# computablee/heterogeneous-spmv

Hardware: AMD Instinct MI355X
Metric: SpMV GFLOP/s and achieved HBM GB/s (fp64) per matrix, 1/2/4/8 MI355X (higher is better)
Workload: dtype f64

## Files before the change

heterogeneous-spmv_amd/csrc/hspmv_options.cpp:

```cpp
#include <string.h>

#include <algorithm>
#include <atomic>
#include <cmath>
#include <cstddef>
#include <cstdlib>
#include <thread>
#include <vector>

#include "hspmv_runtime.h"

namespace hspmv {

int tuning_from_options(const hspmv_options *o, Tuning *t) {
  *t = Tuning();
  if (!o) return HSPMV_OK;
  if (o->struct_size < offsetof(hspmv_options, csr3_plan))
    return set_error(HSPMV_E_INVALID, "hspmv_options.struct_size %u too small", o->struct_size);
  hspmv_options v;
  memset(&v, 0, sizeof(v));
  memcpy(&v, o, std::min<size_t>(o->struct_size, sizeof(v)));
  if (v.csr3_plan < 0 || v.csr3_plan > HSPMV_CSR3_PLAN_SSR)
    return set_error(HSPMV_E_INVALID, "csr3_plan %d unknown", v.csr3_plan);
  if ((v.csort_parts && v.csort_parts != 1 && v.csort_parts != 2 && v.csort_parts != 4) ||
      (v.csort_chunk_u && v.csort_chunk_u != 4 && v.csort_chunk_u != 8 && v.csort_chunk_u != 16) ||
      (v.stream_waves && v.stream_waves != 1 && v.stream_waves != 2 && v.stream_waves != 4) ||
      v.task_nnz < 0 || v.x_dict_cap < 0 || v.placement_trials < 0 || v.placement_trials > 8)
    return set_error(HSPMV_E_INVALID, "hspmv_options: value out of range");
  if (v.deterministic < 0 || v.deterministic > HSPMV_DETERMINISTIC_SERIAL)
    return set_error(HSPMV_E_INVALID, "deterministic %d unknown", v.deterministic);
  if ((v.deterministic == HSPMV_DETERMINISTIC_ORDERED || v.deterministic == HSPMV_DETERMINISTIC_SERIAL) &&
      v.csort > 0)
    return set_error(HSPMV_E_INVALID, "the column-sorted kernel (csort = 1) does not sum in omp_spmv's "
                                      "order (deterministic = 2 runs it with reproducible fixed-point sums)");
  t->csr3_plan = v.csr3_plan;
  t->task_nnz = v.task_nnz;
  t->x_windows = v.x_windows < 0 ? -1 : 0;
  t->x_dict = v.x_dict < 0 ? -1 : (v.x_dict > 0 ? 1 : 0);
  t->x_dict_cap = v.x_dict_cap;
  t->x_slabs = v.x_slabs < 0 ? -1 : v.x_slabs;
  t->col16_group = v.col16_group < 0 ? -1 : (v.col16_group > 0 ? 1 : 0);
  t->csort = v.csort < 0 ? -1 : (v.csort > 0 ? 1 : 0);
  t->csort_parts = v.csort_parts;
  t->csort_u = v.csort_chunk_u;
  t->stream_waves = v.stream_waves;
  t->deterministic = v.deterministic;
  t->placement_trials = v.placement_trials;
  t->row_slices = v.row_slices < 0 ? -1 : (v.row_slices > 0 ? 1 : 0);
  return HSPMV_OK;
}

#ifdef HSPMV_ENV_KNOBS
void tuning_from_env(Tuning *t) {
  auto geti = [](const char *k, int *v) {
    if (const char *e = getenv(k)) *v = atoi(e);
  };
  if (const char *e = getenv("HSPMV_CSR3_PLAN"))
    t->csr3_plan = !strcmp(e, "ssr") ? HSPMV_CSR3_PLAN_SSR
                   : !strcmp(e, "packed") ? HSPMV_CSR3_PLAN_PACKED : HSPMV_CSR3_PLAN_ALIGNED;
  if (const char *e = getenv("HSPMV_TASK_FILL"))
    if (atoi(e) == 0) t->csr3_plan = HSPMV_CSR3_PLAN_PACKED;
  geti("HSPMV_TASK_NNZ", &t->task_nnz);
  if (const char *e = getenv("HSPMV_XWIN")) t->x_windows = atoi(e) == 0 ? -1 : 0;
  if (const char *e = getenv("HSPMV_XDICT")) t->x_dict = atoi(e) == 0 ? -1 : 1;
  geti("HSPMV_XDICT_CAP", &t->x_dict_cap);
  if (const char *e = getenv("HSPMV_XSLABS")) t->x_slabs = atoi(e) == 0 ? -1 : atoi(e);
  if (const char *e = getenv("HSPMV_XSLAB_BYTES")) t->xslab_bytes = atof(e);
  if (const char *e = getenv("HSPMV_COL16G")) t->col16_group = atoi(e) == 0 ? -1 : 1;
  if (const char *e = getenv("HSPMV_CSORT")) t->csort = atoi(e) == 0 ? -1 : 1;
  geti("HSPMV_CSORT_H", &t->csort_parts);
  geti("HSPMV_CSORT_U", &t->csort_u);
// ... 3 lines not shown
  geti("HSPMV_CSORT_SLOT32", &t->csort_slot32);
  geti("HSPMV_CSORT_WIDE", &t->csort_wide);
  geti("HSPMV_CSORT_LDS", &t->csort_lds_cap);
  geti("HSPMV_CSORT_SEG", &t->csort_seg);
  geti("HSPMV_CSORT_SEG_EXTRA", &t->csort_seg_extra);
  geti("HSPMV_CSORT_TRACE", &t->csort_trace);
  geti("HSPMV_CSORT_LONG", &t->csort_long);
  geti("HSPMV_CSORT_BALANCE", &t->csort_balance);
  geti("HSPMV_CSORT_FIN_ROWS", &t->csort_fin_rows);
  geti("HSPMV_CSORT_DYN", &t->csort_dyn);
  if (const char *e = getenv("HSPMV_CSORT_SWEEP")) t->csort_sweep_w = atof(e);
  if (const char *e = getenv("HSPMV_CSORT_SLACK")) t->csort_slack = atof(e);
  geti("HSPMV_CSORT_PART32", &t->csort_part32);
  geti("HSPMV_DETERMINISTIC", &t->deterministic);
  geti("HSPMV_SERIAL_MAX", &t->serial_max);
  geti("HSPMV_LDS_PAD", &t->lds_pad);
  geti("HSPMV_STREAM_W", &t->stream_waves);
  geti("HSPMV_PLACEMENT", &t->placement_trials);
  geti("HSPMV_SSR_ALIGN", &t->ssr_align);
  geti("HSPMV_SSR_W", &t->ssr_w);
  geti("HSPMV_CONTIG", &t->contig);
  geti("HSPMV_XD_WAVES", &t->xd_waves);
  geti("HSPMV_XD_BPC", &t->xd_blocks_per_cu);
  if (const char *e = getenv("HSPMV_ROW_SLICES")) t->row_slices = atoi(e) == 0 ? -1 : 1;
  geti("HSPMV_PF", &t->pf);
  geti("HSPMV_YNT", &t->y_nt);
  geti("HSPMV_NT", &t->nt);
  geti("HSPMV_DYNLDS", &t->dyn_lds);
}
#else
void tuning_from_env(Tuning *) {}
#endif

int check_deterministic(unsigned flags, const Tuning &t) {
  const unsigned k = flag_kernel(flags);
  if ((t.deterministic == HSPMV_DETERMINISTIC_ORDERED || t.deterministic == HSPMV_DETERMINISTIC_SERIAL) &&
      k == kCsort)
    return set_error(HSPMV_E_INVALID, "the column-sorted kernel (HSPMV_KERNEL_CSORT) does not sum in "
                                      "omp_spmv's order (deterministic = 2 runs it with reproducible "
                                      "fixed-point sums)");
  if (t.deterministic == HSPMV_DETERMINISTIC_SERIAL) {
    if (k == kVector)
      return set_error(HSPMV_E_INVALID, "deterministic = 3 (serial order) runs the row kernels only: "
                                        "HSPMV_KERNEL_VECTOR sums each row in a shuffle tree");
  }
  return HSPMV_OK;
}
// ... 9 lines not shown
```

heterogeneous-spmv_amd/csrc/hspmv_slices.cpp:

```cpp
#include <string.h>

#include <algorithm>
#include <cstddef>
#include <vector>

#include "hspmv_runtime.h"

namespace hspmv {


std::vector<int32_t> slice_starts(int kern, int64_t m, const std::vector<int32_t> &tasks) {
  if (kern == kCsr3) return tasks;
  std::vector<int32_t> st;
  for (int64_t r = 0; r < m; r += 64) st.push_back((int32_t)r);
  if (st.empty()) st.push_back(0);
  st.push_back((int32_t)m);
  return st;
}

int slices_why(const Tuning &t, unsigned flags, int kern, int W, const int32_t *rp, int64_t m,
               int64_t n, int dtype, int val_dtype, const std::vector<int32_t> &starts, SliceCounts *out) {
  SliceCounts c;
  c.n_desc = (int64_t)starts.size() - 1;
  for (int64_t s = 0; s < c.n_desc; ++s) {
    const int32_t a = starts[(size_t)s], b = starts[(size_t)s + 1];
// ... 52 lines not shown
  P.desc[2 * (size_t)nd] = (int32_t)pre;
  P.desc[2 * (size_t)nd + 1] = (int32_t)m;
  P.padded = pre;
  P.len.assign((size_t)std::max<int64_t>(m, 1), 0);
  for (int64_t r = 0; r < m; ++r) P.len[(size_t)r] = (uint8_t)(rp[r + 1] - rp[r]);
  P.pos.assign((size_t)std::max<int64_t>(64 * pre, 1), 0);
  P.val.assign(sv * (size_t)std::max<int64_t>(64 * pre, 1), 0);
  parallel_ranges(nd, 256, [&](int64_t s0, int64_t s1, int) {
    for (int64_t s = s0; s < s1; ++s) {
      const int32_t a = starts[(size_t)s], b = starts[(size_t)s + 1];
      const size_t base = 64 * (size_t)P.desc[2 * (size_t)s];
      const int32_t w = P.desc[2 * (size_t)s + 2] - P.desc[2 * (size_t)s];
      for (int32_t r = a; r < b; ++r)
        for (int32_t k = 0; k < rp[r + 1] - rp[r]; ++k) {
          const size_t src = (size_t)rp[r] + (size_t)k;
          P.pos[slot_at(base, w, k, r - a, 4)] = pos[src];
          memcpy(P.val.data() + sv * slot_at(base, w, k, r - a, G), (const char *)val + sv * src, sv);
        }
    }
  });
}

static inline int64_t pos_units(int32_t w, int bits) { return bits == 12 ? 6 * (w / 8) + w % 8 : w; }

static int slice_pos_bits(const int32_t *desc, int64_t nd, const uint16_t *pos) {
  const int64_t n = 64 * (int64_t)desc[2 * nd];
  uint16_t top = 0;
  for (int64_t i = 0; i < n; ++i) top = std::max(top, pos[i]);
  int64_t units12 = 0;
  for (int64_t s = 0; s < nd; ++s) units12 += pos_units(desc[2 * s + 2] - desc[2 * s], 12);
  return top < 4096 && 128 * units12 + 4 * (nd + 1) < 2 * n ? 12 : 16;
}

static void pack_slice_pos(const int32_t *desc, int64_t nd, const uint16_t *pos, int bits, int32_t *prefix,
                    unsigned char *out) {
  int64_t pre = 0;
  for (int64_t s = 0; s < nd; ++s) {
    prefix[s] = (int32_t)pre;
    pre += pos_units(desc[2 * s + 2] - desc[2 * s], bits);
  }
  prefix[nd] = (int32_t)pre;
  if (!out) return;
  if (bits != 12) {
    memcpy(out, pos, 128 * (size_t)pre);
    return;
  }
// ... 6 lines not shown
        for (int i = 0; i < 64; ++i) {
          uint64_t p[8];
          for (int e = 0; e < 8; ++e) p[e] = pos[slot_at(base, w, 8 * g + e, i, 4)];
          const uint64_t lo = p[0] | p[1] << 12 | p[2] << 24 | p[3] << 36 | p[4] << 48 | p[5] << 60;
          const uint32_t d[3] = {(uint32_t)lo, (uint32_t)(lo >> 32),
                                 (uint32_t)(p[5] >> 4 | p[6] << 8 | p[7] << 20)};
          memcpy(dst + 768 * (size_t)g + 12 * (size_t)i, d, 12);
        }
      for (int32_t k = w8; k < w; ++k)
        for (int i = 0; i < 64; ++i) {
          const uint16_t v = pos[slot_at(base, w, k, i, 4)];
          memcpy(dst + 96 * (size_t)w8 + 2 * slot_at(0, w - w8, k - w8, i, 4), &v, 2);
        }
    }
  });
}

int upload_slices(Shard &s, const SlicePlan &P) {
  DevSlices &d = s.built.sl;
  int rc;
  const int64_t nd = (int64_t)P.desc.size() / 2 - 1;
  int32_t bits = 0;
  int64_t stream = 0;
  if ((rc = hspmv_slices_pack(nd, P.desc.data(), P.pos.data(), &bits, &stream, nullptr, nullptr))) return rc;
  size_t pos_bytes = 2 * P.pos.size(), table_bytes = 0;
  if (bits == 12) {
    std::vector<int32_t> prefix((size_t)nd + 1);
    std::vector<unsigned char> packed((size_t)stream + 16, 0);
    if ((rc = hspmv_slices_pack(nd, P.desc.data(), P.pos.data(), &bits, &stream, prefix.data(), packed.data())))
      return rc;
    pos_bytes = packed.size();
    table_bytes = 4 * prefix.size();
    if ((rc = s.dev.upload(&d.pos, packed.data(), pos_bytes))) return rc;
    if ((rc = s.dev.upload(&d.ppre, prefix.data(), table_bytes))) return rc;
  } else if ((rc = s.dev.upload(&d.pos, P.pos.data(), pos_bytes))) {
    return rc;
  }
  if ((rc = s.dev.upload(&d.desc, P.desc.data(), 4 * P.desc.size()))) return rc;
  if ((rc = s.dev.upload(&d.len, P.len.data(), P.len.size()))) return rc;
  if ((rc = s.dev.upload(&d.val, P.val.data(), P.val.size()))) return rc;
  d.n = (int32_t)nd;
  d.pos_bits = bits;
  s.saved.sl_desc_n = nd;
  s.saved.sl_padded = P.padded;
  s.saved.sl_pos_bytes = stream + (int64_t)table_bytes;
  return HSPMV_OK;
}

void drop_slices(Shard &s) {
  const DevSlices &d = s.built.sl;
  for (const void *p : std::initializer_list<const void *>{d.desc, d.len, d.pos, d.ppre, d.val}) s.dev.release(p);
  s.built.sl = DevSlices();
  s.A.has_slices = false;
}

// ... 51 lines not shown
  build_slices(A->row_ptr, P.pos.data(), A->val, A->m, A->dtype, starts, S);
  if (desc) memcpy(desc, S.desc.data(), 4 * S.desc.size());
  if (len && A->m) memcpy(len, S.len.data(), (size_t)A->m);
  if (pos && S.padded) memcpy(pos, S.pos.data(), 2 * (size_t)(64 * S.padded));
  if (val && S.padded) memcpy(val, S.val.data(), dtype_size(A->dtype) * (size_t)(64 * S.padded));
  return HSPMV_OK;
}

int hspmv_slices_pack(int64_t n_desc, const int32_t *desc, const uint16_t *pos, int32_t *bits,
                      int64_t *pos_bytes, int32_t *pos_prefix, void *packed) {
  clear_error();
  if (n_desc < 0 || !desc || !pos || !bits || !pos_bytes) return set_error(HSPMV_E_INVALID, "NULL argument");
  for (int64_t s = 0; s < n_desc; ++s)
    if (desc[2 * s] < 0 || desc[2 * s + 2] < desc[2 * s]) return set_error(HSPMV_E_INVALID, "desc: prefixes decrease");
  *bits = slice_pos_bits(desc, n_desc, pos);
  std::vector<int32_t> prefix((size_t)n_desc + 1);
  pack_slice_pos(desc, n_desc, pos, *bits, prefix.data(), nullptr);
  *pos_bytes = 128 * (int64_t)prefix[(size_t)n_desc];
  if (pos_prefix) memcpy(pos_prefix, prefix.data(), 4 * prefix.size());
  if (packed) pack_slice_pos(desc, n_desc, pos, *bits, prefix.data(), (unsigned char *)packed);
  return HSPMV_OK;
}

}
```

heterogeneous-spmv_amd/csrc/hspmv_xdict.cpp:

```cpp
#include <string.h>

#include <algorithm>
#include <atomic>
#include <cmath>
#include <cstddef>
#include <cstdlib>
#include <vector>

#include "hspmv_runtime.h"

namespace hspmv {

constexpr int32_t kXdGap = 8;
constexpr int32_t kXdMaxRuns = 63;
constexpr int32_t kXdCapBytes = 20 * 1024;

int kernel_for_tables(int64_t n_ssr, bool have_tasks, unsigned flags) {
  const unsigned k = flag_kernel(flags);
  if (k == kVector) return kVector;
  if ((k == kCsr3 || k == kAuto) && n_ssr > 0)
    return have_tasks ? kCsr3 : -1;
  if ((k == kCsr3 || k == kAuto) && have_tasks) return kCsr3;
  return kStream;
}
// ... 145 lines not shown
  return cut;
}

bool plan_xdict_for(const int32_t *rp, const int32_t *col, int kern, int64_t m,
                    std::vector<int32_t> &tasks, int W, int32_t long_t, int64_t cap, int dtype,
                    const Tuning &tune, bool slices, bool fill, XdPlan &P, int64_t *cut) {
  *cut = 0;
  const bool cuts = kern == kCsr3 && W == 4 && tune.csr3_plan != HSPMV_CSR3_PLAN_SSR &&
                    tune.xd_blocks_per_cu >= 0;
  if (!plan_xdict(rp, col, xdict_blocks(kern, m, tasks, W), long_t, cap, fill && !cuts, P))
    return false;
  if (!cuts) return true;
  *cut = split_xd_blocks(tasks, P.total, xd_target_entries(dtype, tune, slices));
  if (*cut == 0 && !fill) return true;
  return plan_xdict(rp, col, xdict_blocks(kern, m, tasks, W), long_t, cap, fill, P);
}

int build_xdict(Shard &s, const int32_t *rp, const int32_t *col, const void *val, int64_t m, int64_t n,
                unsigned flags, bool have_xwin) {
  const int dtype = s.dtype;
  s.xd_shape = 0;
  const int mode = s.tune.x_dict > 0 ? 1 : (s.tune.x_dict < 0 ? 0 : -1);
  if (mode == 0 || (flags & HSPMV_FLAG_NO_COL16) || m == 0) return HSPMV_OK;
  if (mode < 0 && have_xwin) return HSPMV_OK;
  const int kern = kernel_for_tables(s.A.n_ssr, !s.host.tasks.empty(), flags);
  if (kern != kStream && kern != kCsr3) return HSPMV_OK;
  const int W = xd_block_tasks(s.tune, s.A.task_waves);
  if (kern == kCsr3 && W != 4 && W != 8) return HSPMV_OK;
  if (kern == kStream && flag_groups(flags) > 1) return HSPMV_OK;
  const double sv = (double)dtype_size(dtype);
  const int64_t nnz = rp[m];
  if (mode < 0 && mall_resident(m, n, nnz, dtype, s.val_dtype)) return HSPMV_OK;
  const int32_t long_t = split_threshold(flags);
  XdPlan P;
  std::vector<int32_t> tasks = s.host.tasks;
  const bool slices = slices_why(s.tune, flags, kern, W, rp, m, n, dtype, s.val_dtype,
                                 slice_starts(kern, m, tasks), nullptr) == HSPMV_SLICES_OK;
  if (!plan_xdict_for(rp, col, kern, m, tasks, W, long_t, xdict_cap_entries(dtype, s.tune), dtype,
                      s.tune, slices, true, P, &s.xd_cut))
    return HSPMV_OK;
  if (mode < 0 && 2 * P.entries > P.in_kernel_nnz) return HSPMV_OK;
  s.host.tasks.swap(tasks);
  int rc;
  if (slices) {
    SlicePlan S;
    build_slices(rp, P.pos.data(), val, m, s.val_dtype, slice_starts(kern, m, s.host.tasks), S);
    if ((rc = upload_slices(s, S))) return rc;
    s.A.has_slices = true;
  } else if ((rc = s.dev.upload(&s.d_c16, P.pos.data(), 2 * P.pos.size()))) {
    return rc;
  }
  DevXdict &d = s.built.xd;
  if ((rc = s.dev.upload(&d.blk, P.blk.data(), 4 * P.blk.size()))) return rc;
  if ((rc = s.dev.upload(&d.runs, P.rec.data(), 4 * P.rec.size()))) return rc;
  s.A.col16 = slices ? s.built.sl.pos : s.d_c16;
  s.A.cbase = nullptr;
  s.A.cplanes = nullptr;
  s.A.n_cplanes = 0;
  s.xd_shape = kern;
  if (kern == kCsr3) s.A.task_waves = W;
  d.lds_bytes = (int32_t)((int64_t)P.tmax * (int64_t)sv);
  s.saved.xd_entries = P.entries;
  s.saved.xd_runs_n = (int64_t)P.rec.size() / 2;
  return HSPMV_OK;
}

int plan_shape(const hspmv_csr *A, const hspmv_csr3_maps *maps, const hspmv_options *opt, PlanShape &ps) {
  int rc;
  if ((rc = tuning_from_options(opt, &ps.tune))) return rc;
// ... 80 lines not shown
```

heterogeneous-spmv_amd/csrc/row_launch.cuh:

```cuda
#pragma once
#include "row_kernels.cuh"
#include "slice_kernel.cuh"
#include "static_switch.h"

namespace hspmv {
namespace dev {

inline uint32_t block_order(const LaunchPlan &p) {
  return (uint32_t)p.xcd_chunk | (p.reverse ? kSweepReverse : 0u);
}

template <typename T, typename TV>
hipError_t launch_slices(const DevPlan &dp, const LaunchPlan &p, const T *x, T *y, hipStream_t st) {
  if (!dp.xd.blk || !dp.sl.len || !dp.sl.pos || !dp.sl.val || p.waves_per_block != 4 ||
      p.blocks != ((int64_t)dp.sl.n + 3) / 4 ||
      !(dp.sl.pos_bits == 16 || (dp.sl.pos_bits == 12 && dp.sl.ppre)))
    return hipErrorInvalidValue;
  const Slices sl{dp.sl.desc, dp.sl.len, dp.sl.pos, dp.sl.ppre};
  const XDict xd{dp.xd.blk, reinterpret_cast<const int2 *>(dp.xd.runs)};
  const unsigned dyn = (unsigned)dp.xd.lds_bytes + (unsigned)p.dyn_lds;
  const TV *val = static_cast<const TV *>(dp.sl.val);
  static_switch<12, 16>(dp.sl.pos_bits, [&](auto PB) {
    static_flag(p.nontemporal, [&](auto NT) {
      hipLaunchKernelGGL((hspmv_slices<T, NT, HSPMV_SLICE_BATCH, PB, TV>), dim3((unsigned)p.blocks), dim3(256), dyn,
                         st, dp.sl.n, block_order(p), (int32_t)p.y_nt, sl, xd, val, x, y);
    });
  });
  return hipGetLastError();
}

inline ColSrc col_src(const DevCSR &A) {
  return ColSrc{A.col_idx, A.col16, A.cbase, A.cplanes, A.n_cplanes, A.cplane_words};
}

template <typename T, typename TV, bool NT, int U, bool PF, int C16, bool XD>
void launch_rows_shape(const DevCSR &A, const DevPlan &dp, const LaunchPlan &p, const T *x, T *y,
                       hipStream_t st) {
  const TV *val = static_cast<const TV *>(A.val);
  const ColSrc cs = col_src(A);
  const XDict xd{dp.xd.blk, reinterpret_cast<const int2 *>(dp.xd.runs)};
  const int2 *xw = reinterpret_cast<const int2 *>(dp.xwin);
  const unsigned dyn = XD ? (unsigned)dp.xd.lds_bytes + (unsigned)p.dyn_lds : (unsigned)p.dyn_lds;
  const dim3 grid((unsigned)p.blocks);
  const int wpb = p.waves_per_block;
  if (p.kernel == kStream) {
// ... 58 lines not shown
```

heterogeneous-spmv_amd/csrc/slice_kernel.cuh:

```cuda
#pragma once
#include "row_kernels.cuh"

namespace hspmv {
namespace dev {

#ifndef HSPMV_SLICE_BATCH
#define HSPMV_SLICE_BATCH 8
#endif

struct Slices {
  const int32_t *desc;
  const uint8_t *len;
  const uint16_t *pos;
  const int32_t *ppre;
};

typedef int32_t sl_i4 __attribute__((ext_vector_type(4), aligned(4)));
typedef uint32_t sl_u3 __attribute__((ext_vector_type(3), aligned(4)));

template <typename TV, int B>
struct SliceBatch {
  TV v[B];
  uint32_t pq[B / 2];
  uint32_t ps[3];
// ... 10 lines not shown
        pbb(pb + (uint64_t)(uint32_t)k0 * (kWave * PB / 8u)) {}
};

template <typename TV, bool NT, int B, int PB>
__device__ __forceinline__ void slice_load_full(SliceBatch<TV, B> &q, const gchar *vb, const gchar *pb,
                                                int32_t k0, int lane) {
  typedef SliceAt<TV, PB> At;
  constexpr int G = At::G;
  const At at(vb, pb, k0);
#pragma unroll
  for (int j = 0; j < B / G; ++j) {
    const typename At::tv t = ld_off<NT, typename At::tv>(at.vbb, (uint32_t)(j * kWave + lane) * 16u);
#pragma unroll
    for (int e = 0; e < G; ++e) q.v[j * G + e] = t[e];
  }
  if constexpr (PB == 12) {
#pragma unroll
    for (int g = 0; g < B / 8; ++g) {
      const sl_u3 t = ld_off<NT, sl_u3>(at.pbb, (uint32_t)(g * kWave + lane) * 12u);
      q.pq[3 * g] = t[0];
      q.pq[3 * g + 1] = t[1];
      q.pq[3 * g + 2] = t[2];
    }
  } else {
#pragma unroll
    for (int g = 0; g < B / 4; ++g) {
      const typename At::u2 t = ld_off<NT, typename At::u2>(at.pbb, (uint32_t)(g * kWave + lane) * 8u);
      q.pq[2 * g] = t[0];
      q.pq[2 * g + 1] = t[1];
    }
  }
}

template <typename TV, bool NT, int B, int PB>
__device__ __forceinline__ void slice_load_tail(SliceBatch<TV, B> &q, const gchar *vb, const gchar *pb,
                                                int32_t k0, int32_t w, int lane) {
  typedef SliceAt<TV, PB> At;
  constexpr int G = At::G;
  const At at(vb, pb, k0);
#pragma unroll
  for (int i = 0; i < B; ++i) q.v[i] = TV(0);
#pragma unroll
  for (int i = 0; i < B / 2; ++i) q.pq[i] = 0u;
#pragma unroll
  for (int i = 0; i < 3; ++i) q.ps[i] = 0u;
#pragma unroll
  for (int j = 0; j < B / G; ++j) {
    if (k0 + j * G + G <= w) {
      const typename At::tv t = ld_off<NT, typename At::tv>(at.vbb, (uint32_t)(j * kWave + lane) * 16u);
#pragma unroll
      for (int e = 0; e < G; ++e) q.v[j * G + e] = t[e];
    } else {
#pragma unroll
      for (int e = 0; e < G - 1; ++e)
        if (k0 + j * G + e < w)
          q.v[j * G + e] = ld_off<NT, TV>(at.vbb, (uint32_t)((j * G + e) * kWave + lane) * (uint32_t)sizeof(TV));
    }
  }
#pragma unroll
  for (int g = 0; g < B / 4; ++g) {
    if (k0 + 4 * g + 4 <= w) {
      const typename At::u2 t = ld_off<NT, typename At::u2>(at.pbb, (uint32_t)(g * kWave + lane) * 8u);
      q.pq[2 * g] = t[0];
      q.pq[2 * g + 1] = t[1];
    } else {
#pragma unroll
      for (int r = 0; r < 3; ++r)
        if (k0 + 4 * g + r < w)
          q.ps[r] = (uint32_t)ld_off<NT, uint16_t>(at.pbb, (uint32_t)((4 * g + r) * kWave + lane) * 2u);
    }
  }
}

template <int PB>
__device__ __forceinline__ uint32_t slice_pos(const uint32_t *pq, int i) {
  if constexpr (PB == 12) {
    const int d = 3 * (i / 8) + 12 * (i % 8) / 32, sh = 12 * (i % 8) % 32;
    uint32_t v = pq[d] >> sh;
    if (sh > 20) v |= pq[d + 1] << (32 - sh);
    return v & 0xfffu;
  } else {
    return (pq[i / 2] >> (16 * (i & 1))) & 0xffffu;
  }
}

template <typename T, int B, int PB, typename TV>
__device__ __forceinline__ T slice_consume(T acc, const SliceBatch<TV, B> &q, const T *xs, int32_t k0,
                                           int32_t w, int32_t len, bool full) {
  T xv[B];
#pragma unroll
  for (int i = 0; i < B; ++i) {
    const int g = i / 4, r = i % 4;
    const uint32_t p = (full || k0 + 4 * g + 4 <= w) ? slice_pos<PB>(q.pq, i) : q.ps[r < 3 ? r : 0];
    xv[i] = xs[p];
  }
#pragma unroll
  for (int i = 0; i < B; ++i) {
    const T p = (T)q.v[i] * xv[i];
    acc = (k0 + i < len) ? acc + p : acc;
  }
  return acc;
}

template <typename T, bool NT, int B, int PB, typename TV = T>
__global__ __launch_bounds__(256) void hspmv_slices(int32_t n_slices, uint32_t blk_order, int32_t y_nt,
                                                    Slices sl, XDict xd, const TV *__restrict__ val,
                                                    const T *__restrict__ x, T *__restrict__ y) {
  static_assert(B % 4 == 0 && B >= 4, "batches hold whole position groups");
  static_assert(PB == 16 || (PB == 12 && B % 8 == 0), "12-bit positions come in groups of 8 slots");
  static_assert(B % (16 / (int)sizeof(TV)) == 0, "batches hold whole 16-byte value groups");
  extern __shared__ __attribute__((aligned(16))) unsigned char xdyn[];
  const int wid = threadIdx.x >> 6;
  const int lane = threadIdx.x & (kWave - 1);
  const int64_t blk = sweep_block(blockIdx.x, gridDim.x, blk_order);
  const int64_t t = blk * 4 + wid;
  int32_t off = 0, poff = 0, w = 0, r0 = 0, nr = 0;
  if (t < n_slices) {
    const sl_i4 d = sload<sl_i4, 4>(sl.desc, (uint64_t)t * 8u);
    off = d[0];
    r0 = d[1];
    w = d[2] - d[0];
    nr = d[3] - d[1];
    poff = PB == 12 ? sload<int32_t>(sl.ppre, (uint64_t)t * 4u) : off;
  }
  int32_t len = 0;
  if (lane < nr) len = (int32_t)sl.len[r0 + lane];
  stage_xdict<T, 256>(reinterpret_cast<T *>(xdyn), x, xd, blk, threadIdx.x);
  if (nr <= 0) return;
  const T *xs = reinterpret_cast<const T *>(xdyn);
  const gchar *vb = uniform_ptr(val + (int64_t)off * kWave);
  const gchar *pb = uniform_ptr(sl.pos + (int64_t)poff * kWave);
  const int32_t wf = w & ~(B - 1);
  T acc = T(0);
  SliceBatch<TV, B> cur, nxt, tail;
  int32_t k0 = 0;
  if (wf > 0) slice_load_full<TV, NT, B, PB>(cur, vb, pb, 0, lane);
  for (; k0 + 3 * B <= wf; k0 += 2 * B) {
    slice_load_full<TV, NT, B, PB>(nxt, vb, pb, k0 + B, lane);
    __builtin_amdgcn_sched_barrier(0);
    acc = slice_consume<T, B, PB>(acc, cur, xs, k0, w, len, true);
    __builtin_amdgcn_sched_barrier(0);
    slice_load_full<TV, NT, B, PB>(cur, vb, pb, k0 + 2 * B, lane);
    __builtin_amdgcn_sched_barrier(0);
    acc = slice_consume<T, B, PB>(acc, nxt, xs, k0 + B, w, len, true);
    __builtin_amdgcn_sched_barrier(0);
  }
  if (k0 + 2 * B <= wf) {
    slice_load_full<TV, NT, B, PB>(nxt, vb, pb, k0 + B, lane);
    __builtin_amdgcn_sched_barrier(0);
    acc = slice_consume<T, B, PB>(acc, cur, xs, k0, w, len, true);
    __builtin_amdgcn_sched_barrier(0);
    cur = nxt;
    k0 += B;
  }
  if (w > wf) slice_load_tail<TV, NT, B, PB>(tail, vb, pb, wf, w, lane);
  __builtin_amdgcn_sched_barrier(0);
  if (wf > 0) acc = slice_consume<T, B, PB>(acc, cur, xs, wf - B, w, len, true);
  if (w > wf) acc = slice_consume<T, B, 16>(acc, tail, xs, wf, w, len, false);
  if constexpr (diag(kDiagNoStore)) {
    if (lane < nr && acc == T(12345.678)) y[r0 + lane] = acc;
  } else if (lane < nr) {
    if (y_nt)
      __builtin_nontemporal_store(acc, y + r0 + lane);
    else
      y[r0 + lane] = acc;
  }
}

}
}
```

heterogeneous-spmv_amd/hspmv/__init__.py:

```python
from ._lib import HspmvError, LIB_PATH, lib
from .api import (Csr3Maps, CsrMatrix, SpMM, SpMV, alg_bytes, build_csr2_bandk, build_csr2_maps,
                  build_csr3_bandk, build_csr3_maps,
                  csr3_params, device_count, load_bin, partition_rows, rcm_reorder, read_csr,
                  read_csr3, read_mtx, save_bin, version, write_csr, write_csr3, xdict_plan, slices_plan, slices_pack, values_fit_float32)

__all__ = ["HspmvError", "LIB_PATH", "lib", "Csr3Maps", "CsrMatrix", "SpMM", "SpMV", "alg_bytes",
           "build_csr2_bandk", "build_csr2_maps", "build_csr3_bandk", "build_csr3_maps", "csr3_params", "device_count", "load_bin", "partition_rows",
           "rcm_reorder", "read_csr", "read_csr3", "read_mtx", "save_bin", "version", "write_csr", "write_csr3", "xdict_plan", "slices_plan", "slices_pack", "values_fit_float32"]
```

heterogeneous-spmv_amd/hspmv/_lib.py:

```python
from __future__ import annotations

import ctypes as C
import os
from pathlib import Path

PKG_ROOT = Path(__file__).resolve().parent.parent
REPO_ROOT = PKG_ROOT.parent
LIB_PATH = Path(os.environ.get("HSPMV_LIB", PKG_ROOT / "build" / "libhspmv.so.1"))
HEADER = REPO_ROOT / "include" / "hspmv.h"

F32, F64 = 0, 1

KERNEL_AUTO, KERNEL_VECTOR, KERNEL_STREAM, KERNEL_CSR3, KERNEL_CSORT = 0, 1, 2, 3, 4
LANES_SHIFT = 4
FLAG_NO_COL16 = 1 << 11
FLAG_NONTEMPORAL = 1 << 12
FLAG_DEVICE_PTRS = 1 << 13
FLAG_NO_XCD_REMAP = 1 << 14
FLAG_NO_SPLIT = 1 << 15
U_SHIFT = 16
FLAG_PREFETCH = 1 << 21
FLAG_XCD_REMAP = 1 << 22
FLAG_COL16 = 1 << 23
XCD_CHUNK_SHIFT = 24
# ... 199 lines not shown
    "hspmv_save_bin": (C.c_int, [C.c_char_p, C.POINTER(Csr), C.POINTER(Csr3Maps)]),
    "hspmv_load_bin": (C.c_int, [C.c_char_p, C.POINTER(CsrBuf), C.POINTER(Csr3Buf)]),
    "hspmv_free_csr": (None, [C.POINTER(CsrBuf)]),
    "hspmv_free_csr3": (None, [C.POINTER(Csr3Buf)]),
    "hspmv_build_csr3_maps": (C.c_int, [C.POINTER(Csr), C.c_int, C.c_int, C.POINTER(Csr3Buf)]),
    "hspmv_build_csr3_bandk": (C.c_int, [C.POINTER(Csr), C.c_int, C.c_int, C.POINTER(CsrBuf),
                                         C.POINTER(Csr3Buf), _P]),
    "hspmv_build_csr2_maps": (C.c_int, [C.POINTER(Csr), C.c_int, C.POINTER(Csr3Buf)]),
    "hspmv_build_csr2_bandk": (C.c_int, [C.POINTER(Csr), C.c_int, C.POINTER(CsrBuf),
                                         C.POINTER(Csr3Buf), _P]),
    "hspmv_csr3_params": (C.c_int, [C.c_double, C.c_int, C.POINTER(C.c_int), C.POINTER(C.c_int)]),
    "hspmv_partition_rows": (C.c_int, [C.c_int64, _P, C.POINTER(Csr3Maps), C.c_int, _P]),
    "hspmv_xdict_plan_ex": (C.c_int, [C.POINTER(Csr), C.POINTER(Csr3Maps), C.POINTER(Options), C.c_int64,
                                      C.POINTER(C.c_int64), C.POINTER(C.c_int64), _P, _P, _P]),
    "hspmv_xdict_plan": (C.c_int, [C.POINTER(Csr), C.POINTER(Csr3Maps), C.c_uint, C.c_int64,
                                   C.POINTER(C.c_int64), C.POINTER(C.c_int64), _P, _P, _P]),
    "hspmv_slices_plan": (C.c_int, [C.POINTER(Csr), C.POINTER(Csr3Maps), C.POINTER(Options),
                                    C.POINTER(C.c_int64), C.POINTER(C.c_int64), C.POINTER(C.c_int64),
                                    C.POINTER(C.c_int32), _P, _P, _P, _P]),
    "hspmv_slices_plan_vec": (C.c_int, [C.POINTER(Csr), C.POINTER(Csr3Maps), C.POINTER(Options), C.c_int,
                                        C.POINTER(C.c_int64), C.POINTER(C.c_int64), C.POINTER(C.c_int64),
                                        C.POINTER(C.c_int32), _P, _P, _P, _P]),
    "hspmv_slices_pack": (C.c_int, [C.c_int64, _P, _P, C.POINTER(C.c_int32), C.POINTER(C.c_int64), _P, _P]),
    "hspmv_alg_bytes": (C.c_double, [C.c_int64, C.c_int64, C.c_int64, C.c_int, C.c_int64, C.c_int64]),
    "hspmv_device_count": (C.c_int, [C.POINTER(C.c_int)]),
    "hspmv_rccl_version": (C.c_int, [C.POINTER(C.c_int)]),
    "hspmv_last_error": (C.c_char_p, []),
    "hspmv_version": (C.c_char_p, []),
}

_LIB = None


def lib() -> C.CDLL:
    global _LIB
    if _LIB is None:
        if not LIB_PATH.exists():
            raise RuntimeError(
                f"libhspmv.so not found at {LIB_PATH}: build it with "
                f"`make -C {PKG_ROOT}` or `python -c 'import __graft_entry__ as g; g.build()'`")
        handle = C.CDLL(str(LIB_PATH))
        for name, (res, args) in SIGNATURES.items():
            fn = getattr(handle, name)
            fn.restype = res
            fn.argtypes = args
        _LIB = handle
# ... 12 lines not shown
```

heterogeneous-spmv_amd/hspmv/api.py:

```python
from __future__ import annotations

import ctypes as C
from dataclasses import dataclass, field
from typing import Optional

import numpy as np

from . import _lib
from ._lib import (F32, F64, KERNEL_AUTO, KERNEL_CSORT, KERNEL_CSR3, KERNEL_STREAM, KERNEL_VECTOR,
                   FLAG_DEVICE_PTRS, FLAG_NONTEMPORAL, HspmvError, check, lanes_flag, lib,
                   remap_flag)

_KERNELS = {"auto": KERNEL_AUTO, "vector": KERNEL_VECTOR, "stream": KERNEL_STREAM,
            "csr3": KERNEL_CSR3, "csort": KERNEL_CSORT}
KERNEL_NAMES = {v: k for k, v in _KERNELS.items()}


def dtype_code(dtype) -> int:
    dt = np.dtype(dtype)
    if dt == np.float64:
        return F64
    if dt == np.float32:
        return F32
    raise ValueError(f"unsupported dtype {dt} (float32 / float64)")
# ... 276 lines not shown
    rl = np.zeros(max(A.m, 1), np.uint8)
    pos = np.zeros(max(pe.value, 1), np.uint16)
    val = np.zeros(max(pe.value, 1), A.val.dtype)
    check(plan_fn(*args, _ptr(desc), _ptr(rl), _ptr(pos), _ptr(val)), "slices_plan")
    out.update(desc=desc, len=rl[:A.m], pos=pos[:pe.value], val=val[:pe.value],
               n_desc=nd.value)
    return out


def slices_pack(desc: np.ndarray, pos: np.ndarray) -> dict:
    desc = np.ascontiguousarray(desc, dtype=np.int32).reshape(-1, 2)
    pos = np.ascontiguousarray(pos, dtype=np.uint16)
    nd = desc.shape[0] - 1
    if nd < 0 or pos.shape[0] < 64 * int(desc[nd, 0]):
        raise ValueError("slices_pack: pos is shorter than desc's 64 * total width")
    bits, nbytes = C.c_int32(), C.c_int64()
    L = lib()
    args = (nd, _ptr(desc), _ptr(pos), C.byref(bits), C.byref(nbytes))
    check(L.hspmv_slices_pack(*args, None, None), "slices_pack")
    prefix = np.empty(nd + 1, np.int32)
    packed = np.zeros(max(nbytes.value, 1), np.uint8)
    check(L.hspmv_slices_pack(*args, _ptr(prefix), _ptr(packed)), "slices_pack")
    return {"bits": bits.value, "pos_prefix": prefix, "packed": packed[:nbytes.value]}


def alg_bytes(m: int, n: int, nnz: int, dtype, n_ssr: int = 0, n_sr: int = 0) -> float:
    return float(lib().hspmv_alg_bytes(m, n, nnz, dtype_code(dtype), n_ssr, n_sr))


def device_count() -> int:
    c = C.c_int()
    rc = lib().hspmv_device_count(C.byref(c))
    return c.value if rc == 0 else 0


def version() -> str:
    return lib().hspmv_version().decode()



def _check_values(val, nnz: int, dtype) -> np.ndarray:
    val = np.asarray(val)
    if val.shape != (nnz,):
        raise ValueError(f"val has shape {val.shape}, expected (nnz,) = ({nnz},)")
    if not np.can_cast(val.dtype, dtype, casting="same_kind"):
        raise ValueError(f"val has dtype {val.dtype}, which does not cast to {np.dtype(dtype)}")
# ... 309 lines not shown
```

include/hspmv.h:

```cpp
#ifndef HSPMV_H
#define HSPMV_H

#include <stdint.h>

#ifdef __cplusplus
extern "C" {
#endif

#define HSPMV_VERSION_MAJOR 1
#define HSPMV_VERSION_MINOR 1

#define HSPMV_OK 0
#define HSPMV_E_INVALID (-1)
#define HSPMV_E_IO (-2)
#define HSPMV_E_NOMEM (-3)
#define HSPMV_E_HIP (-4)
#define HSPMV_E_RCCL (-5)
#define HSPMV_E_NODEV (-6)
#define HSPMV_E_STATE (-7)

typedef enum { HSPMV_F32 = 0, HSPMV_F64 = 1 } hspmv_dtype;

typedef struct {
  int64_t m, n, nnz;
// ... 241 lines not shown
int hspmv_xdict_plan_ex(const hspmv_csr *A, const hspmv_csr3_maps *maps, const hspmv_options *opt,
                        int64_t cap_entries, int64_t *n_blocks, int64_t *n_records,
                        int32_t *blk, int32_t *runs, uint16_t *pos);
int hspmv_xdict_plan(const hspmv_csr *A, const hspmv_csr3_maps *maps, unsigned flags,
                     int64_t cap_entries, int64_t *n_blocks, int64_t *n_records,
                     int32_t *blk, int32_t *runs, uint16_t *pos);
#define HSPMV_SLICES_OK 0
#define HSPMV_SLICES_OFF 1
#define HSPMV_SLICES_NO_DICT 2
#define HSPMV_SLICES_SHAPE 3
#define HSPMV_SLICES_CHUNKED 4
#define HSPMV_SLICES_SPLIT_ROWS 5
#define HSPMV_SLICES_LONG_ROW 6
#define HSPMV_SLICES_BYTES 7
#define HSPMV_SLICES_RESIDENT 8
int hspmv_slices_plan(const hspmv_csr *A, const hspmv_csr3_maps *maps, const hspmv_options *opt,
                      int64_t *n_desc, int64_t *n_slices, int64_t *padded_entries, int32_t *why,
                      int32_t *desc, uint8_t *len, uint16_t *pos, void *val);
int hspmv_slices_plan_vec(const hspmv_csr *A, const hspmv_csr3_maps *maps, const hspmv_options *opt,
                          int vector_dtype, int64_t *n_desc, int64_t *n_slices, int64_t *padded_entries,
                          int32_t *why, int32_t *desc, uint8_t *len, uint16_t *pos, void *val);
int hspmv_slices_pack(int64_t n_desc, const int32_t *desc, const uint16_t *pos, int32_t *bits,
                      int64_t *pos_bytes, int32_t *pos_prefix, void *packed);
double hspmv_alg_bytes(int64_t m, int64_t n, int64_t nnz, int dtype,
                       int64_t n_ssr, int64_t n_sr);
int hspmv_device_count(int *count);
int hspmv_rccl_version(int *version);
const char *hspmv_last_error(void);
const char *hspmv_version(void);

#ifdef __cplusplus
}
#endif
#endif
```

Baseline: 1212.

## Add 8-bit per-slice base-offset position encoding for sliced x-dictionary SpMV

```diff
diff --git a/heterogeneous-spmv_amd/csrc/hspmv_options.cpp b/heterogeneous-spmv_amd/csrc/hspmv_options.cpp
--- a/heterogeneous-spmv_amd/csrc/hspmv_options.cpp
+++ b/heterogeneous-spmv_amd/csrc/hspmv_options.cpp
@@ -46,7 +46,7 @@
   t->stream_waves = v.stream_waves;
   t->deterministic = v.deterministic;
   t->placement_trials = v.placement_trials;
-  t->row_slices = v.row_slices < 0 ? -1 : (v.row_slices > 0 ? 1 : 0);
+  t->row_slices = v.row_slices < 0 ? -1 : std::min(v.row_slices, 2);
   return HSPMV_OK;
 }
 
@@ -96,7 +96,7 @@
   geti("HSPMV_CONTIG", &t->contig);
   geti("HSPMV_XD_WAVES", &t->xd_waves);
   geti("HSPMV_XD_BPC", &t->xd_blocks_per_cu);
-  if (const char *e = getenv("HSPMV_ROW_SLICES")) t->row_slices = atoi(e) == 0 ? -1 : 1;
+  if (const char *e = getenv("HSPMV_ROW_SLICES")) t->row_slices = atoi(e) == 0 ? -1 : std::min(atoi(e), 2);
   geti("HSPMV_PF", &t->pf);
   geti("HSPMV_YNT", &t->y_nt);
   geti("HSPMV_NT", &t->nt);
diff --git a/heterogeneous-spmv_amd/csrc/hspmv_slices.cpp b/heterogeneous-spmv_amd/csrc/hspmv_slices.cpp
--- a/heterogeneous-spmv_amd/csrc/hspmv_slices.cpp
+++ b/heterogeneous-spmv_amd/csrc/hspmv_slices.cpp
@@ -1,6 +1,8 @@
 #include <string.h>
 
 #include <algorithm>
+#include <atomic>
+#include <climits>
 #include <cstddef>
 #include <vector>
 
@@ -99,6 +101,59 @@
 }
 
 static inline int64_t pos_units(int32_t w, int bits) { return bits == 12 ? 6 * (w / 8) + w % 8 : w; }
+
+static inline size_t slot8_at(int32_t w, int32_t k, int i) {
+  const int32_t w8 = w / 8 * 8;
+  if (k < w8) return (size_t)(k / 8) * 512 + (size_t)i * 8 + (size_t)(k % 8);
+  if (w - w8 >= 4 && k - w8 < 4) return (size_t)w8 * 64 + (size_t)i * 4 + (size_t)(k - w8);
+  return (size_t)k * 64 + (size_t)i;
+}
+
+static bool slice_span(const int32_t *desc, int64_t s, const uint8_t *len, const uint16_t *pos, int32_t *lo,
+                       int32_t *hi) {
+  const size_t base = 64 * (size_t)desc[2 * s];
+  const int32_t w = desc[2 * s + 2] - desc[2 * s], r0 = desc[2 * s + 1];
+  const int32_t nr = std::min<int32_t>(desc[2 * s + 3] - r0, 64);
+  int32_t a = INT32_MAX, b = -1;
+  for (int32_t i = 0; i < nr; ++i)
+    for (int32_t k = 0; k < std::min<int32_t>(len[r0 + i], w); ++k) {
+      const int32_t p = pos[slot_at(base, w, k, i, 4)];
+      a = std::min(a, p);
+      b = std::max(b, p);
+    }
+  *lo = a;
+  *hi = b;
+  return b >= 0;
+}
+
+static bool slice_pos8_fits(const int32_t *desc, int64_t nd, const uint8_t *len, const uint16_t *pos) {
+  std::atomic<bool> fits{true};
+  parallel_ranges(nd, 256, [&](int64_t s0, int64_t s1, int) {
+    for (int64_t s = s0; s < s1 && fits.load(std::memory_order_relaxed); ++s) {
+      int32_t lo, hi;
+      if (slice_span(desc, s, len, pos, &lo, &hi) && hi - lo > 255) fits = false;
+    }
+  });
+  return fits;
+}
+
+static void pack_slice_pos8(const int32_t *desc, int64_t nd, const uint8_t *len, const uint16_t *pos,
+                            int32_t *base, unsigned char *out) {
+  if (out) memset(out, 0, 64 * (size_t)desc[2 * nd]);
+  parallel_ranges(nd, 256, [&](int64_t s0, int64_t s1, int) {
+    for (int64_t s = s0; s < s1; ++s) {
+      int32_t lo, hi;
+      base[s] = slice_span(desc, s, len, pos, &lo, &hi) ? lo : 0;
+      if (!out) continue;
+      const size_t at = 64 * (size_t)desc[2 * s];
+      const int32_t w = desc[2 * s + 2] - desc[2 * s], r0 = desc[2 * s + 1];
+      const int32_t nr = std::min<int32_t>(desc[2 * s + 3] - r0, 64);
+      for (int32_t i = 0; i < nr; ++i)
+        for (int32_t k = 0; k < std::min<int32_t>(len[r0 + i], w); ++k)
+          out[at + slot8_at(w, k, i)] = (unsigned char)(pos[slot_at(at, w, k, i, 4)] - base[s]);
+    }
+  });
+}
 
 static int slice_pos_bits(const int32_t *desc, int64_t nd, const uint16_t *pos) {
   const int64_t n = 64 * (int64_t)desc[2 * nd];
@@ -151,15 +206,19 @@
   const int64_t nd = (int64_t)P.desc.size() / 2 - 1;
   int32_t bits = 0;
   int64_t stream = 0;
-  if ((rc = hspmv_slices_pack(nd, P.desc.data(), P.pos.data(), &bits, &stream, nullptr, nullptr))) return rc;
+  const int narrowest = s.tune.row_slices == 1 ? 12 : 8;
+  if ((rc = hspmv_slices_pack_ex(nd, P.desc.data(), P.len.data(), P.pos.data(), narrowest, &bits, &stream, nullptr,
+                                 nullptr)))
+    return rc;
   size_t pos_bytes = 2 * P.pos.size(), table_bytes = 0;
-  if (bits == 12) {
+  if (bits != 16) {
     std::vector<int32_t> prefix((size_t)nd + 1);
     std::vector<unsigned char> packed((size_t)stream + 16, 0);
-    if ((rc = hspmv_slices_pack(nd, P.desc.data(), P.pos.data(), &bits, &stream, prefix.data(), packed.data())))
+    if ((rc = hspmv_slices_pack_ex(nd, P.desc.data(), P.len.data(), P.pos.data(), narrowest, &bits, &stream,
+                                   prefix.data(), packed.data())))
       return rc;
     pos_bytes = packed.size();
-    table_bytes = 4 * prefix.size();
+    table_bytes = 4 * (prefix.size() - (bits == 8 ? 1 : 0));
     if ((rc = s.dev.upload(&d.pos, packed.data(), pos_bytes))) return rc;
     if ((rc = s.dev.upload(&d.ppre, prefix.data(), table_bytes))) return rc;
   } else if ((rc = s.dev.upload(&d.pos, P.pos.data(), pos_bytes))) {
@@ -257,4 +316,25 @@
   return HSPMV_OK;
 }
 
-}
+int hspmv_slices_pack_ex(int64_t n_desc, const int32_t *desc, const uint8_t *len, const uint16_t *pos,
+                         int narrowest_bits, int32_t *bits, int64_t *pos_bytes, int32_t *table, void *packed) {
+  clear_error();
+  if (narrowest_bits != 8 && narrowest_bits != 12)
+    return set_error(HSPMV_E_INVALID, "narrowest_bits %d (8 or 12)", narrowest_bits);
+  if (n_desc < 0 || !desc || !len || !pos || !bits || !pos_bytes) return set_error(HSPMV_E_INVALID, "NULL argument");
+  for (int64_t s = 0; s < n_desc; ++s)
+    if (desc[2 * s] < 0 || desc[2 * s + 2] < desc[2 * s] || desc[2 * s + 1] < 0 || desc[2 * s + 3] < desc[2 * s + 1])
+      return set_error(HSPMV_E_INVALID, "desc: prefixes or rows decrease");
+  if (narrowest_bits == 8 && slice_pos8_fits(desc, n_desc, len, pos)) {
+    *bits = 8;
+    *pos_bytes = 64 * (int64_t)desc[2 * n_desc];
+    if (!table && !packed) return HSPMV_OK;
+    std::vector<int32_t> base((size_t)n_desc + 1, 0);
+    pack_slice_pos8(desc, n_desc, len, pos, base.data(), (unsigned char *)packed);
+    if (table) memcpy(table, base.data(), 4 * base.size());
+    return HSPMV_OK;
+  }
+  return hspmv_slices_pack(n_desc, desc, pos, bits, pos_bytes, table, packed);
+}
+
+}
diff --git a/heterogeneous-spmv_amd/csrc/hspmv_xdict.cpp b/heterogeneous-spmv_amd/csrc/hspmv_xdict.cpp
--- a/heterogeneous-spmv_amd/csrc/hspmv_xdict.cpp
+++ b/heterogeneous-spmv_amd/csrc/hspmv_xdict.cpp
@@ -191,7 +191,9 @@
   s.xd_shape = 0;
   const int mode = s.tune.x_dict > 0 ? 1 : (s.tune.x_dict < 0 ? 0 : -1);
   if (mode == 0 || (flags & HSPMV_FLAG_NO_COL16) || m == 0) return HSPMV_OK;
-  if (mode < 0 && have_xwin) return HSPMV_OK;
+  const bool over_xwin = mode < 0 && have_xwin;
+  if (over_xwin && (s.tune.row_slices < 0 || s.tune.row_slices == 1 || s.tune.placement_trials > 1))
+    return HSPMV_OK;
   const int kern = kernel_for_tables(s.A.n_ssr, !s.host.tasks.empty(), flags);
   if (kern != kStream && kern != kCsr3) return HSPMV_OK;
   const int W = xd_block_tasks(s.tune, s.A.task_waves);
@@ -205,15 +207,30 @@
   std::vector<int32_t> tasks = s.host.tasks;
   const bool slices = slices_why(s.tune, flags, kern, W, rp, m, n, dtype, s.val_dtype,
                                  slice_starts(kern, m, tasks), nullptr) == HSPMV_SLICES_OK;
+  if (over_xwin && !slices) return HSPMV_OK;
   if (!plan_xdict_for(rp, col, kern, m, tasks, W, long_t, xdict_cap_entries(dtype, s.tune), dtype,
                       s.tune, slices, true, P, &s.xd_cut))
     return HSPMV_OK;
   if (mode < 0 && 2 * P.entries > P.in_kernel_nnz) return HSPMV_OK;
+  SlicePlan S;
+  if (slices) build_slices(rp, P.pos.data(), val, m, s.val_dtype, slice_starts(kern, m, tasks), S);
+  if (over_xwin) {
+    const int64_t nd = (int64_t)S.desc.size() / 2 - 1, ng = kern == kCsr3 ? (int64_t)tasks.size() - 1 : (m + 63) / 64;
+    const double sval = (double)dtype_size(s.val_dtype);
+    int32_t bits = 0;
+    int64_t stream = 0;
+    if (hspmv_slices_pack_ex(nd, S.desc.data(), S.len.data(), S.pos.data(), 8, &bits, &stream, nullptr, nullptr) ||
+        bits != 8 ||
+        64.0 * (double)S.padded * sval + (double)stream + (double)m + 8.0 * (double)(nd + 1) + 4.0 * (double)nd +
+                4.0 * (double)(P.rec.size() + P.blk.size()) >=
+            (double)nnz * (sval + 2.0) + 4.0 * (double)(m + 1) + 8.0 * (double)ng) {
+      s.xd_cut = 0;
+      return HSPMV_OK;
+    }
+  }
   s.host.tasks.swap(tasks);
   int rc;
   if (slices) {
-    SlicePlan S;
-    build_slices(rp, P.pos.data(), val, m, s.val_dtype, slice_starts(kern, m, s.host.tasks), S);
     if ((rc = upload_slices(s, S))) return rc;
     s.A.has_slices = true;
   } else if ((rc = s.dev.upload(&s.d_c16, P.pos.data(), 2 * P.pos.size()))) {
diff --git a/heterogeneous-spmv_amd/csrc/row_launch.cuh b/heterogeneous-spmv_amd/csrc/row_launch.cuh
--- a/heterogeneous-spmv_amd/csrc/row_launch.cuh
+++ b/heterogeneous-spmv_amd/csrc/row_launch.cuh
@@ -14,13 +14,13 @@
 hipError_t launch_slices(const DevPlan &dp, const LaunchPlan &p, const T *x, T *y, hipStream_t st) {
   if (!dp.xd.blk || !dp.sl.len || !dp.sl.pos || !dp.sl.val || p.waves_per_block != 4 ||
       p.blocks != ((int64_t)dp.sl.n + 3) / 4 ||
-      !(dp.sl.pos_bits == 16 || (dp.sl.pos_bits == 12 && dp.sl.ppre)))
+      !(dp.sl.pos_bits == 16 || ((dp.sl.pos_bits == 12 || dp.sl.pos_bits == 8) && dp.sl.ppre)))
     return hipErrorInvalidValue;
   const Slices sl{dp.sl.desc, dp.sl.len, dp.sl.pos, dp.sl.ppre};
   const XDict xd{dp.xd.blk, reinterpret_cast<const int2 *>(dp.xd.runs)};
   const unsigned dyn = (unsigned)dp.xd.lds_bytes + (unsigned)p.dyn_lds;
   const TV *val = static_cast<const TV *>(dp.sl.val);
-  static_switch<12, 16>(dp.sl.pos_bits, [&](auto PB) {
+  static_switch<8, 12, 16>(dp.sl.pos_bits, [&](auto PB) {
     static_flag(p.nontemporal, [&](auto NT) {
       hipLaunchKernelGGL((hspmv_slices<T, NT, HSPMV_SLICE_BATCH, PB, TV>), dim3((unsigned)p.blocks), dim3(256), dyn,
                          st, dp.sl.n, block_order(p), (int32_t)p.y_nt, sl, xd, val, x, y);
diff --git a/heterogeneous-spmv_amd/csrc/slice_kernel.cuh b/heterogeneous-spmv_amd/csrc/slice_kernel.cuh
--- a/heterogeneous-spmv_amd/csrc/slice_kernel.cuh
+++ b/heterogeneous-spmv_amd/csrc/slice_kernel.cuh
@@ -56,6 +56,13 @@
       q.pq[3 * g + 1] = t[1];
       q.pq[3 * g + 2] = t[2];
     }
+  } else if constexpr (PB == 8) {
+#pragma unroll
+    for (int g = 0; g < B / 8; ++g) {
+      const typename At::u2 t = ld_off<NT, typename At::u2>(at.pbb, (uint32_t)(g * kWave + lane) * 8u);
+      q.pq[2 * g] = t[0];
+      q.pq[2 * g + 1] = t[1];
+    }
   } else {
 #pragma unroll
     for (int g = 0; g < B / 4; ++g) {
@@ -93,7 +100,16 @@
   }
 #pragma unroll
   for (int g = 0; g < B / 4; ++g) {
-    if (k0 + 4 * g + 4 <= w) {
+    if constexpr (PB == 8) {
+      if (g == 0 && k0 + 4 <= w) {
+        q.pq[0] = ld_off<NT, uint32_t>(at.pbb, (uint32_t)lane * 4u);
+      } else {
+#pragma unroll
+        for (int r = 0; r < 3; ++r)
+          if (k0 + 4 * g + r < w)
+            q.ps[r] = (uint32_t)ld_off<NT, uint8_t>(at.pbb, (uint32_t)((4 * g + r) * kWave + lane));
+      }
+    } else if (k0 + 4 * g + 4 <= w) {
       const typename At::u2 t = ld_off<NT, typename At::u2>(at.pbb, (uint32_t)(g * kWave + lane) * 8u);
       q.pq[2 * g] = t[0];
       q.pq[2 * g + 1] = t[1];
@@ -113,6 +129,8 @@
     uint32_t v = pq[d] >> sh;
     if (sh > 20) v |= pq[d + 1] << (32 - sh);
     return v & 0xfffu;
+  } else if constexpr (PB == 8) {
+    return (pq[i / 4] >> (8 * (i & 3))) & 0xffu;
   } else {
     return (pq[i / 2] >> (16 * (i & 1))) & 0xffffu;
   }
@@ -141,7 +159,8 @@
                                                     Slices sl, XDict xd, const TV *__restrict__ val,
                                                     const T *__restrict__ x, T *__restrict__ y) {
   static_assert(B % 4 == 0 && B >= 4, "batches hold whole position groups");
-  static_assert(PB == 16 || (PB == 12 && B % 8 == 0), "12-bit positions come in groups of 8 slots");
+  static_assert(PB == 16 || (PB == 12 && B % 8 == 0) || (PB == 8 && B == 8),
+                "12- and 8-bit positions come in groups of 8 slots");
   static_assert(B % (16 / (int)sizeof(TV)) == 0, "batches hold whole 16-byte value groups");
   extern __shared__ __attribute__((aligned(16))) unsigned char xdyn[];
   const int wid = threadIdx.x >> 6;
@@ -155,15 +174,16 @@
     r0 = d[1];
     w = d[2] - d[0];
     nr = d[3] - d[1];
-    poff = PB == 12 ? sload<int32_t>(sl.ppre, (uint64_t)t * 4u) : off;
+    poff = PB != 16 ? sload<int32_t>(sl.ppre, (uint64_t)t * 4u) : off;
   }
   int32_t len = 0;
   if (lane < nr) len = (int32_t)sl.len[r0 + lane];
   stage_xdict<T, 256>(reinterpret_cast<T *>(xdyn), x, xd, blk, threadIdx.x);
   if (nr <= 0) return;
-  const T *xs = reinterpret_cast<const T *>(xdyn);
+  const T *xs = reinterpret_cast<const T *>(xdyn) + (PB == 8 ? poff : 0);
   const gchar *vb = uniform_ptr(val + (int64_t)off * kWave);
-  const gchar *pb = uniform_ptr(sl.pos + (int64_t)poff * kWave);
+  const gchar *pb = PB == 8 ? uniform_ptr(reinterpret_cast<const uint8_t *>(sl.pos) + (int64_t)off * kWave)
+                            : uniform_ptr(sl.pos + (int64_t)poff * kWave);
   const int32_t wf = w & ~(B - 1);
   T acc = T(0);
   SliceBatch<TV, B> cur, nxt, tail;
@@ -190,7 +210,7 @@
   if (w > wf) slice_load_tail<TV, NT, B, PB>(tail, vb, pb, wf, w, lane);
   __builtin_amdgcn_sched_barrier(0);
   if (wf > 0) acc = slice_consume<T, B, PB>(acc, cur, xs, wf - B, w, len, true);
-  if (w > wf) acc = slice_consume<T, B, 16>(acc, tail, xs, wf, w, len, false);
+  if (w > wf) acc = slice_consume<T, B, PB == 8 ? 8 : 16>(acc, tail, xs, wf, w, len, false);
   if constexpr (diag(kDiagNoStore)) {
     if (lane < nr && acc == T(12345.678)) y[r0 + lane] = acc;
   } else if (lane < nr) {
diff --git a/heterogeneous-spmv_amd/hspmv/__init__.py b/heterogeneous-spmv_amd/hspmv/__init__.py
--- a/heterogeneous-spmv_amd/hspmv/__init__.py
+++ b/heterogeneous-spmv_amd/hspmv/__init__.py
@@ -2,8 +2,8 @@
 from .api import (Csr3Maps, CsrMatrix, SpMM, SpMV, alg_bytes, build_csr2_bandk, build_csr2_maps,
                   build_csr3_bandk, build_csr3_maps,
                   csr3_params, device_count, load_bin, partition_rows, rcm_reorder, read_csr,
-                  read_csr3, read_mtx, save_bin, version, write_csr, write_csr3, xdict_plan, slices_plan, slices_pack, values_fit_float32)
+                  read_csr3, read_mtx, save_bin, version, write_csr, write_csr3, xdict_plan, slices_plan, slices_pack, slices_pack_ex, values_fit_float32)
 
 __all__ = ["HspmvError", "LIB_PATH", "lib", "Csr3Maps", "CsrMatrix", "SpMM", "SpMV", "alg_bytes",
            "build_csr2_bandk", "build_csr2_maps", "build_csr3_bandk", "build_csr3_maps", "csr3_params", "device_count", "load_bin", "partition_rows",
-           "rcm_reorder", "read_csr", "read_csr3", "read_mtx", "save_bin", "version", "write_csr", "write_csr3", "xdict_plan", "slices_plan", "slices_pack", "values_fit_float32"]
+           "rcm_reorder", "read_csr", "read_csr3", "read_mtx", "save_bin", "version", "write_csr", "write_csr3", "xdict_plan", "slices_plan", "slices_pack", "slices_pack_ex", "values_fit_float32"]
diff --git a/heterogeneous-spmv_amd/hspmv/_lib.py b/heterogeneous-spmv_amd/hspmv/_lib.py
--- a/heterogeneous-spmv_amd/hspmv/_lib.py
+++ b/heterogeneous-spmv_amd/hspmv/_lib.py
@@ -245,6 +245,8 @@
                                         C.POINTER(C.c_int64), C.POINTER(C.c_int64), C.POINTER(C.c_int64),
                                         C.POINTER(C.c_int32), _P, _P, _P, _P]),
     "hspmv_slices_pack": (C.c_int, [C.c_int64, _P, _P, C.POINTER(C.c_int32), C.POINTER(C.c_int64), _P, _P]),
+    "hspmv_slices_pack_ex": (C.c_int, [C.c_int64, _P, _P, _P, C.c_int, C.POINTER(C.c_int32),
+                                       C.POINTER(C.c_int64), _P, _P]),
     "hspmv_alg_bytes": (C.c_double, [C.c_int64, C.c_int64, C.c_int64, C.c_int, C.c_int64, C.c_int64]),
     "hspmv_device_count": (C.c_int, [C.POINTER(C.c_int)]),
     "hspmv_rccl_version": (C.c_int, [C.POINTER(C.c_int)]),
diff --git a/heterogeneous-spmv_amd/hspmv/api.py b/heterogeneous-spmv_amd/hspmv/api.py
--- a/heterogeneous-spmv_amd/hspmv/api.py
+++ b/heterogeneous-spmv_amd/hspmv/api.py
@@ -322,6 +322,27 @@
     packed = np.zeros(max(nbytes.value, 1), np.uint8)
     check(L.hspmv_slices_pack(*args, _ptr(prefix), _ptr(packed)), "slices_pack")
     return {"bits": bits.value, "pos_prefix": prefix, "packed": packed[:nbytes.value]}
+
+
+def slices_pack_ex(desc: np.ndarray, rl: np.ndarray, pos: np.ndarray, narrowest: int = 8) -> dict:
+    desc = np.ascontiguousarray(desc, dtype=np.int32).reshape(-1, 2)
+    rl = np.ascontiguousarray(rl, dtype=np.uint8)
+    pos = np.ascontiguousarray(pos, dtype=np.uint16)
+    nd = desc.shape[0] - 1
+    if nd < 0 or pos.shape[0] < 64 * int(desc[nd, 0]):
+        raise ValueError("slices_pack_ex: pos is shorter than desc's 64 * total width")
+    if rl.shape[0] < int(desc[nd, 1]):
+        raise ValueError("slices_pack_ex: len is shorter than desc's rows")
+    bits, nbytes = C.c_int32(), C.c_int64()
+    L = lib()
+    args = (nd, _ptr(desc), _ptr(rl) if rl.shape[0] else _ptr(np.zeros(1, np.uint8)), _ptr(pos), int(narrowest),
+            C.byref(bits), C.byref(nbytes))
+    check(L.hspmv_slices_pack_ex(*args, None, None), "slices_pack_ex")
+    table = np.empty(nd + 1, np.int32)
+    packed = np.zeros(max(nbytes.value, 1), np.uint8)
+    check(L.hspmv_slices_pack_ex(*args, _ptr(table), _ptr(packed)), "slices_pack_ex")
+    return {"bits": bits.value, "table": table[:nd] if bits.value == 8 else table,
+            "packed": packed[:nbytes.value]}
 
 
 def alg_bytes(m: int, n: int, nnz: int, dtype, n_ssr: int = 0, n_sr: int = 0) -> float:
diff --git a/include/hspmv.h b/include/hspmv.h
--- a/include/hspmv.h
+++ b/include/hspmv.h
@@ -287,6 +287,9 @@
                           int32_t *why, int32_t *desc, uint8_t *len, uint16_t *pos, void *val);
 int hspmv_slices_pack(int64_t n_desc, const int32_t *desc, const uint16_t *pos, int32_t *bits,
                       int64_t *pos_bytes, int32_t *pos_prefix, void *packed);
+int hspmv_slices_pack_ex(int64_t n_desc, const int32_t *desc, const uint8_t *len, const uint16_t *pos,
+                         int narrowest_bits, int32_t *bits, int64_t *pos_bytes, int32_t *table,
+                         void *packed);
 double hspmv_alg_bytes(int64_t m, int64_t n, int64_t nnz, int dtype,
                        int64_t n_ssr, int64_t n_sr);
 int hspmv_device_count(int *count);
```

Result: no change. 1207 (-0.4%).
